# meta-pytorch/torchx

Measured on AMD Instinct MI355X. Metric: tokens_per_second, higher is better.
Workload: dtype bf16; 1 GPU; model=llama3_8b, global_batch=4, seq_len=4096, parallelism=dp1

## Files before the change

torchx_amd/ops/__init__.py:

```python

from __future__ import annotations

import importlib.util
import math
from pathlib import Path
from typing import Optional, Tuple

import torch

from . import reference

_SO = Path(__file__).resolve().parent / "_hip_ops.so"
_hip = None
_load_err: Optional[str] = None


def _load():
    global _hip, _load_err
    if _hip is not None:
        return _hip
    if not _SO.exists():
        _load_err = f"{_SO} not built (run torchx_amd/ops/build.py)"
        return None
    try:
# ... 152 lines not shown
        wt = (hip.transpose_bf16(w)
              if w.shape[0] % 64 == 0 and w.shape[1] % 64 == 0 else None)
        for s in range(0, T, chunk):
            e = min(T, s + chunk)
            x_c = x2[s:e]
            t_c = targets[s:e].contiguous()
            logits_c = x_c @ w.t()
            loss_c, lse_c = hip.ce_fwd(logits_c, t_c)
            loss_sum += loss_c.sum()
            dlog_c = hip.ce_bwd(logits_c, t_c, lse_c, gscale[:e - s])
            if wt is not None:
                torch.matmul(dlog_c, wt.t(), out=dx[s:e])
            else:
                torch.matmul(dlog_c, w, out=dx[s:e])
            if single:
                dw_acc = dlog_c.t() @ x_c
            else:
                dw_acc += dlog_c.t() @ x_c
        ctx.save_for_backward(dx, dw_acc)
        return loss_sum * inv_t

    @staticmethod
    def backward(ctx, gout: torch.Tensor):
        dx, dw_acc = ctx.saved_tensors
        if dw_acc.dtype == dx.dtype:
            dw = dw_acc * gout.to(dx.dtype)
        else:
            dw = (dw_acc * gout.to(torch.float32)).to(dx.dtype)
        dx = dx * gout.to(dx.dtype)
        return dx, dw, None, None


def fused_linear_cross_entropy(
    x: torch.Tensor, w: torch.Tensor, targets: torch.Tensor,
    chunk: int = 16384,
) -> torch.Tensor:
    H = x.shape[-1]
    x2 = x.reshape(-1, H)
    t = targets.reshape(-1)
    if _on_gpu(x):
        if torch.is_grad_enabled() and (x.requires_grad or w.requires_grad):
            return _FusedLinearCE.apply(x2.contiguous(), w, t, chunk)
        hip = hip_ops()
        x2 = x2.contiguous()
        T = x2.shape[0]
        loss_sum = torch.zeros((), device=x.device, dtype=torch.float32)
        for s in range(0, T, chunk):
            e = min(T, s + chunk)
            loss_c, _ = hip.ce_fwd(x2[s:e] @ w.t(), t[s:e].contiguous())
            loss_sum += loss_c.sum()
        return loss_sum / T
    return reference.cross_entropy(x2 @ w.t(), t)




class _FlashAttention(torch.autograd.Function):
    @staticmethod
    def forward(ctx, q: torch.Tensor, k: torch.Tensor, v: torch.Tensor,
                causal: bool, scale: float):
        o, lse = hip_ops().attn_fwd(
            q.contiguous(), k.contiguous(), v.contiguous(), scale, causal
        )
        ctx.save_for_backward(q, k, v, o, lse)
        ctx.causal = causal
        ctx.scale = scale
        return o

    @staticmethod
    def backward(ctx, dout: torch.Tensor):
        q, k, v, o, lse = ctx.saved_tensors
        dq, dk, dv = hip_ops().attn_bwd(
            q, k, v, o, dout.contiguous(), lse, ctx.scale, ctx.causal
        )
        return dq, dk, dv, None, None


def set_attn_bwd_dq_mode(mode: str) -> None:
    hip_ops().set_attn_bwd_dq_mode(mode)


def get_attn_bwd_dq_mode() -> str:
    return hip_ops().get_attn_bwd_dq_mode()


def flash_attention(
    q: torch.Tensor, k: torch.Tensor, v: torch.Tensor,
    causal: bool = True, scale: Optional[float] = None,
) -> torch.Tensor:
    if scale is None:
        scale = 1.0 / math.sqrt(q.shape[-1])
    if _on_gpu(q):
        return _FlashAttention.apply(q, k, v, causal, scale)
    return reference.attention(q, k, v, causal=causal, scale=scale)




def adamw_step(
    p32: torch.Tensor, p16: torch.Tensor, grad: torch.Tensor,
    m: torch.Tensor, v: torch.Tensor, *, lr: float, beta1: float = 0.9,
    beta2: float = 0.95, eps: float = 1e-8, weight_decay: float = 0.1,
    step: int = 1,
) -> None:
    if p32.is_cuda:
        hip_ops().adamw_step(p32, p16, grad, m, v, lr, beta1, beta2, eps,
                             weight_decay, step)
    else:
        reference.adamw_step(p32, p16, grad, m, v, lr=lr, beta1=beta1,
                             beta2=beta2, eps=eps, weight_decay=weight_decay,
                             step=step)


def mfma_probe(a: torch.Tensor, b: torch.Tensor) -> torch.Tensor:
    return hip_ops().mfma_probe(a, b)




class _FastLinear(torch.autograd.Function):
    @staticmethod
    def forward(ctx, x: torch.Tensor, w: torch.Tensor):
        ctx.save_for_backward(x, w)
        return x @ w.t()

    @staticmethod
    def backward(ctx, dy: torch.Tensor):
        x, w = ctx.saved_tensors
        hip = hip_ops()
        wt = hip.transpose_bf16(w)
        dy2 = dy.reshape(-1, dy.shape[-1]).contiguous()
        x2 = x.reshape(-1, x.shape[-1])
        dx = (dy2 @ wt.t()).view_as(x)
        M, N = dy2.shape
        via_t = N <= 8192 and M % 64 == 0 and N % 64 == 0
        wg = w.grad if w.is_leaf else None
        if wg is not None and wg.is_contiguous():
            a = hip.transpose_bf16(dy2) if via_t else dy2.t()
            if getattr(w, "_wgrad_fresh", False):
                torch.matmul(a, x2, out=wg)
                w._wgrad_fresh = False
            else:
                wg.addmm_(a, x2)
            from torchx_amd.parallel.ddp import grad_ready

            grad_ready(w)
            return dx, None
        dw = (hip.transpose_bf16(dy2) @ x2) if via_t else (dy2.t() @ x2)
        return dx, dw


def fast_linear(x: torch.Tensor, w: torch.Tensor) -> torch.Tensor:
    if (x.is_cuda and w.dtype == torch.bfloat16
            and w.shape[0] % 64 == 0 and w.shape[1] % 64 == 0):
        return _FastLinear.apply(x, w)
    return torch.nn.functional.linear(x, w)




class _FusedAttentionQKV(torch.autograd.Function):
    @staticmethod
    def forward(ctx, qkv: torch.Tensor, cos: torch.Tensor, sin: torch.Tensor,
                Hq: int, Hkv: int, causal: bool, scale: float):
        hip = hip_ops()
        roped = hip.rope_qkv(qkv.contiguous(), cos, sin, Hq, Hkv, 1.0, False)
# ... 200 lines not shown
```

torchx_amd/ops/csrc/attention.hip:

```cpp
#include "common.h"

typedef __bf16 mbf16x8 __attribute__((ext_vector_type(8)));

#define HD 128
#define QBLK 32
#define KBLK 32
#define NWAVES 4
#define BLOCK_Q (QBLK * NWAVES)
#define BLOCK_K (KBLK * NWAVES)

__device__ __forceinline__ f32x16 mfma32(mbf16x8 a, mbf16x8 b, f32x16 c) {
  return __builtin_amdgcn_mfma_f32_32x32x16_bf16(a, b, c, 0, 0, 0);
}

__device__ __forceinline__ unsigned int pack_bf16x2(float a, float b) {
  unsigned int r;
  asm("v_cvt_pk_bf16_f32 %0, %1, %2" : "=v"(r) : "v"(a), "v"(b));
  return r;
}

__device__ __forceinline__ int c_row(int r, int half) {
  return (r & 3) + 8 * (r >> 2) + 4 * half;
}

__device__ __forceinline__ void cvals_to_frags(const float* p, bool hi,
                                               mbf16x8* f0, mbf16x8* f1) {
  unsigned int w[2][4];
  #pragma unroll
  for (int s = 0; s < 2; ++s) {
    unsigned int a01 = pack_bf16x2(p[8 * s + 0], p[8 * s + 1]);
    unsigned int a23 = pack_bf16x2(p[8 * s + 2], p[8 * s + 3]);
    unsigned int a45 = pack_bf16x2(p[8 * s + 4], p[8 * s + 5]);
    unsigned int a67 = pack_bf16x2(p[8 * s + 6], p[8 * s + 7]);
    unsigned int x01 = __shfl_xor((int)a01, 32, 64);
    unsigned int x23 = __shfl_xor((int)a23, 32, 64);
    unsigned int x45 = __shfl_xor((int)a45, 32, 64);
    unsigned int x67 = __shfl_xor((int)a67, 32, 64);
    w[s][0] = hi ? x45 : a01;
    w[s][1] = hi ? x67 : a23;
    w[s][2] = hi ? a45 : x01;
    w[s][3] = hi ? a67 : x23;
  }
  uint4_v u0 = {w[0][0], w[0][1], w[0][2], w[0][3]};
  uint4_v u1 = {w[1][0], w[1][1], w[1][2], w[1][3]};
  *f0 = __builtin_bit_cast(mbf16x8, u0);
  *f1 = __builtin_bit_cast(mbf16x8, u1);
}


#define FKV 64
#define KIMG_BYTES (FKV * 256)
#define VIMG_BYTES (HD * FKV * 2)
#define LOG2E 1.44269504088896340736f
#define LN2 0.69314718055994530942f

__device__ __forceinline__ mbf16x8 kimg_frag(const char* kimg, int sub, int c) {
  const int lane = threadIdx.x & 63;
  const int row = sub * 32 + (lane & 31);
  const int byte = (c * 32 + ((lane >> 5) * 16)) ^ ((row & 15) << 4);
  return *(const mbf16x8*)(kimg + row * 256 + byte);
}

__device__ __forceinline__ int vrot(int d) {
  return ((d >> 1) ^ (d >> 4)) & 7;
}

__device__ __forceinline__ mbf16x8 vimg_frag(const char* vimg, int dt, int ks) {
  const int lane = threadIdx.x & 63;
  const int d = dt * 32 + (lane & 31);
  const int g = (ks * 2 + (lane >> 5) + vrot(d)) & 7;
  return *(const mbf16x8*)(vimg + d * 128 + g * 16);
}

typedef short short4_v __attribute__((ext_vector_type(4)));
typedef __attribute__((address_space(3))) short4_v* lds_s4p;

__device__ __forceinline__ mbf16x8 nat_tr_frag(const char* nat, int ks,
                                               int dt) {
  const int lane = threadIdx.x & 63;
  const int j = lane & 15;
  const int r_lo = ks * 16 + ((lane >> 5) * 8) + (j >> 2);
  const int r_hi = r_lo + 4;
  const int d0 = dt * 32 + ((lane >> 4) & 1) * 16 + 4 * (j & 3);
// ... 811 lines not shown
              s2 = -3.0e38f;
            }
          }
          const float pr =
              __builtin_amdgcn_exp2f(s2 - lse_cur[ql]);
          cv[r] = is_dk ? scale * pr * (acc_dp[r] - del_cur[ql]) : pr;
        }

        mbf16x8 f0, f1;
        cvals_to_frags(cv, hi, &f0, &f1);

        const char* acc_img = is_dk ? qn_c : don_c;
        #pragma unroll
        for (int dt = 0; dt < 4; ++dt) {
          acc[dt] =
              mfma32(f0, nat_tr_frag(acc_img, 2 * sb, dt), acc[dt]);
          acc[dt] =
              mfma32(f1, nat_tr_frag(acc_img, 2 * sb + 1, dt), acc[dt]);
          if (dt == 0) {
            __builtin_amdgcn_sched_barrier(0);
            if (ds_on && qs0 < S) {
              char* p = ds_head +
                        (ds_qt_base(qs0 / BLOCK_Q, ds_nqt, causal) * 4 +
                         ((qs0 / QBLK) & 3)) * DS_IMG_BYTES;
              *(uint4_v*)p = __builtin_bit_cast(uint4_v, f0);
              *(uint4_v*)(p + 32) = __builtin_bit_cast(uint4_v, f1);
              n_ds = 2;
            }
          }
        }
      }
    }

    if (has_next) {
      if (n_ds) {
        asm volatile("s_waitcnt vmcnt(2)" ::: "memory");
      } else {
        asm volatile("s_waitcnt vmcnt(0)" ::: "memory");
      }
      stage_lse(ngh, t0 + (idx + 1) % nt_eff, lse_nxt);
      __syncthreads();
      lse_cur = lse_buf[lse_nxt];
      del_cur = del_buf[lse_nxt];
      lse_nxt ^= 1;
      char* tp;
      tp = qn_c; qn_c = qn_n; qn_n = tp;
      tp = don_c; don_c = don_n; don_n = tp;
    }
  }

  unsigned short* out = is_dk ? dk : dv;
  __syncthreads();
  float* tr = (float*)smem + wave * (32 * 36);
  if (wave_active) {
    #pragma unroll
    for (int dt = 0; dt < 4; ++dt) {
      __syncthreads();
      #pragma unroll
      for (int r = 0; r < 16; ++r) {
        tr[c_row(r, hi) * 36 + kr] = acc[dt][r];
      }
      __syncthreads();
      #pragma unroll
      for (int rep = 0; rep < 4; ++rep) {
        const int kk = kr;
        const int d0 = (hi ? 16 : 0) + rep * 4;
        if (kw0 + kk < S) {
          bf16x4_raw w;
          #pragma unroll
          for (int j = 0; j < 4; ++j) {
            w[j] = (short)f32_to_bf16(tr[kk * 36 + d0 + j]);
          }
          *(bf16x4_raw*)(out + ((long)b * S + kw0 + kk) * out_rs +
                         (long)hkv * HD + dt * 32 + d0) = w;
        }
      }
    }
  } else {
    #pragma unroll
    for (int i = 0; i < 8; ++i) __syncthreads();
  }
}

extern "C" void attn_fwd_launch(const void* q, const void* k, const void* v,
                                void* o, void* lse, int B, int S, int Hq,
                                int Hkv, float scale, int causal,
                                long q_rs, long kv_rs, hipStream_t stream) {
  static int fwd8 = -1;
  if (fwd8 < 0) {
    const char* e = getenv("TORCHX_AMD_FWD_8WAVE");
    fwd8 = (e && atoi(e)) ? 1 : 0;
  }
  if (fwd8 == 1) {
    const int nqt = (S + 8 * QBLK - 1) / (8 * QBLK);
    hipLaunchKernelGGL((attn_fwd_kernel<8>), dim3(B * Hq * nqt), dim3(512),
                       0, stream, (const unsigned short*)q,
                       (const unsigned short*)k, (const unsigned short*)v,
                       (unsigned short*)o, (float*)lse, B, S, Hq, Hkv,
                       scale, causal, q_rs, kv_rs);
  } else {
    const int nqt = (S + 4 * QBLK - 1) / (4 * QBLK);
    hipLaunchKernelGGL((attn_fwd_kernel<4>), dim3(B * Hq * nqt), dim3(256),
                       0, stream, (const unsigned short*)q,
                       (const unsigned short*)k, (const unsigned short*)v,
                       (unsigned short*)o, (float*)lse, B, S, Hq, Hkv,
                       scale, causal, q_rs, kv_rs);
  }
}

extern "C" void attn_bwd_launch(const void* q, const void* k, const void* v,
                                const void* o, const void* dout,
                                const void* lse, void* delta, void* dq,
                                void* dk, void* dv, void* ds, int B, int S,
                                int Hq, int Hkv, float scale, int causal,
                                long q_rs, long kv_rs, long dqkv_q_rs,
                                long dqkv_kv_rs, hipStream_t stream) {
  const long rows = (long)B * S * Hq;
  hipLaunchKernelGGL(attn_bwd_pre_kernel, dim3((int)((rows + 15) / 16)),
                     dim3(256), 0, stream, (const unsigned short*)dout,
                     (const unsigned short*)o, (float*)delta, rows, S, Hq);
  const int nkt = (S + BLOCK_K - 1) / BLOCK_K;
  const long dout_rs = (long)Hq * HD;
  static int dkv_fkv = -1;
  if (dkv_fkv < 0) {
    const char* e = getenv("TORCHX_AMD_DKV_FKV");
    dkv_fkv = (e && atoi(e) == 64) ? 64 : 128;
  }
  if (dkv_fkv == 128 && S % 128 == 0) {
    hipLaunchKernelGGL((attn_bwd_dkv_kernel<128>), dim3(B * Hkv * nkt),
                       dim3(512), 0, stream, (const unsigned short*)q,
                       (const unsigned short*)k, (const unsigned short*)v,
                       (const unsigned short*)dout, (const float*)lse,
                       (const float*)delta, (unsigned short*)dk,
                       (unsigned short*)dv, (char*)ds, B, S, Hq, Hkv,
                       scale, causal, q_rs, kv_rs, dout_rs, dqkv_kv_rs);
  } else {
    hipLaunchKernelGGL((attn_bwd_dkv_kernel<64>), dim3(B * Hkv * nkt),
                       dim3(512), 0, stream, (const unsigned short*)q,
                       (const unsigned short*)k, (const unsigned short*)v,
                       (const unsigned short*)dout, (const float*)lse,
                       (const float*)delta, (unsigned short*)dk,
                       (unsigned short*)dv, (char*)ds, B, S, Hq, Hkv,
                       scale, causal, q_rs, kv_rs, dout_rs, dqkv_kv_rs);
  }
  const int nqt = (S + BLOCK_Q - 1) / BLOCK_Q;
  if (ds != nullptr) {
    static int heavy_first = -1;
    if (heavy_first < 0) {
      const char* e = getenv("TORCHX_AMD_DQ_HEAVY_FIRST");
      heavy_first = (e && atoi(e) == 0) ? 0 : 1;
    }
    hipLaunchKernelGGL(attn_bwd_dq_stream_kernel, dim3(B * Hq * nqt),
                       dim3(256), 0, stream, (const unsigned short*)k,
                       (const char*)ds, (unsigned short*)dq, B, S, Hq, Hkv,
                       causal, kv_rs, dqkv_q_rs, heavy_first);
    return;
  }
  static int dq_fkv = -1;
  if (dq_fkv < 0) {
    const char* e = getenv("TORCHX_AMD_DQ_FKV");
    dq_fkv = (e && atoi(e) == 128) ? 128 : 64;
  }
  if (dq_fkv == 128 && S % 128 == 0) {
    hipLaunchKernelGGL((attn_bwd_dq_kernel<128>), dim3(B * Hq * nqt),
                       dim3(256), 0, stream, (const unsigned short*)q,
                       (const unsigned short*)k, (const unsigned short*)v,
                       (const unsigned short*)dout, (const float*)lse,
                       (const float*)delta, (unsigned short*)dq, B, S, Hq,
                       Hkv, scale, causal, q_rs, kv_rs, dqkv_q_rs);
  } else {
    hipLaunchKernelGGL((attn_bwd_dq_kernel<64>), dim3(B * Hq * nqt),
                       dim3(256), 0, stream, (const unsigned short*)q,
                       (const unsigned short*)k, (const unsigned short*)v,
                       (const unsigned short*)dout, (const float*)lse,
                       (const float*)delta, (unsigned short*)dq, B, S, Hq,
                       Hkv, scale, causal, q_rs, kv_rs, dqkv_q_rs);
  }
}
```

torchx_amd/ops/csrc/bindings.cpp:

```cpp
#include <torch/extension.h>
#include <c10/hip/HIPStream.h>

#include <hip/hip_runtime.h>

extern "C" {
void rope_launch(const void*, void*, const void*, const void*, long, int, int,
                 int, float, hipStream_t);
void swiglu_fwd_launch(const void*, const void*, void*, long, hipStream_t);
void swiglu_bwd_launch(const void*, const void*, const void*, void*, void*,
                       long, hipStream_t);
void rmsnorm_fwd_launch(const void*, const void*, void*, void*, long, int,
                        float, hipStream_t);
void rmsnorm_bwd_launch(const void*, const void*, const void*, const void*,
                        void*, void*, void*, long, int, hipStream_t);
long rmsnorm_bwd_dw_chunks(long);
void adamw_launch(void*, void*, const void*, void*, void*, long, float, float,
                  float, float, float, float, float, hipStream_t);
void ce_fwd_launch(const void*, const void*, void*, void*, long, int,
                   hipStream_t);
void ce_bwd_launch(const void*, const void*, const void*, const void*, void*,
                   long, int, hipStream_t);
void attn_fwd_launch(const void*, const void*, const void*, void*, void*, int,
                     int, int, int, float, int, long, long, hipStream_t);
void attn_bwd_launch(const void*, const void*, const void*, const void*,
                     const void*, const void*, void*, void*, void*, void*,
                     void*, int, int, int, int, float, int, long, long, long,
                     long, hipStream_t);
long attn_bwd_ds_bytes(int, int, int, int);
void rope_qkv_launch(const void*, void*, const void*, const void*, long, int,
                     long, int, float, hipStream_t);
void swiglu_gu_fwd_launch(const void*, void*, long, long, hipStream_t);
void swiglu_gu_bwd_launch(const void*, const void*, void*, long, long,
                          hipStream_t);
void mfma_probe_launch(const void*, const void*, void*, hipStream_t);
void mfma_probe_tr_launch(const void*, const void*, void*, void*,
                          hipStream_t);
void fp8_cast_transpose_launch(const void*, void*, void*, void*,
                               const void*, long, long, int, hipStream_t);
void transpose_bf16_launch(const void*, void*, long, long, hipStream_t);
void decode_attn_launch(const void*, const void*, const void*, void*,
                        const void*, int, int, int, int, int, int, float,
                        hipStream_t);
void gemv_bf16_launch(const void*, const void*, void*, int, int, int,
                      hipStream_t);
void decode_attn_split_launch(const void*, const void*, const void*, void*,
                              void*, void*, const void*, int, int, int, int,
                              int, int, int, float, hipStream_t);
void decode_rope_cache_launch(const void*, void*, void*, void*, const void*,
                              const void*, const void*, int, int, int, int,
                              int, int, hipStream_t);
void rmsnorm_res_launch(const void*, const void*, const void*, void*, void*,
                        long, int, float, hipStream_t);
void gemv_swiglu_launch(const void*, const void*, void*, int, int, int,
                        hipStream_t);
void paged_decode_attn_launch(const void*, const void*, const void*, void*,
                              void*, void*, const void*, const void*, int,
                              int, int, int, int, int, int, float,
                              hipStream_t);
void paged_decode_rope_cache_launch(const void*, void*, void*, void*,
                                    const void*, const void*, const void*,
                                    const void*, int, int, int, int, int,
                                    int, int, hipStream_t);
}

namespace {

hipStream_t cur_stream() {
  return c10::hip::getCurrentHIPStream().stream();
}

void check_bf16(const at::Tensor& t, const char* name) {
  TORCH_CHECK(t.is_cuda(), name, " must be on GPU");
  TORCH_CHECK(t.scalar_type() == at::kBFloat16, name, " must be bf16");
  TORCH_CHECK(t.is_contiguous(), name, " must be contiguous");
}

void check_f32(const at::Tensor& t, const char* name) {
  TORCH_CHECK(t.is_cuda(), name, " must be on GPU");
  TORCH_CHECK(t.scalar_type() == at::kFloat, name, " must be f32");
  TORCH_CHECK(t.is_contiguous(), name, " must be contiguous");
}

}

std::vector<at::Tensor> rmsnorm_fwd(at::Tensor x, at::Tensor w, double eps) {
  check_bf16(x, "x");
  check_bf16(w, "w");
  const long H = x.size(-1);
  TORCH_CHECK(H % 2048 == 0 && H <= 8192, "rmsnorm: H must be k*2048, <=8192");
  const long rows = x.numel() / H;
  auto y = at::empty_like(x);
  auto invrms = at::empty({rows}, x.options().dtype(at::kFloat));
  rmsnorm_fwd_launch(x.data_ptr(), w.data_ptr(), y.data_ptr(),
                     invrms.data_ptr(), rows, (int)H, (float)eps,
                     cur_stream());
  return {y, invrms};
}

std::vector<at::Tensor> rmsnorm_bwd(at::Tensor dy, at::Tensor x, at::Tensor w,
                                    at::Tensor invrms) {
  check_bf16(dy, "dy");
  check_bf16(x, "x");
  const long H = x.size(-1);
  TORCH_CHECK(H % 2048 == 0 && H <= 8192, "rmsnorm: H must be k*2048, <=8192");
  const long rows = x.numel() / H;
  auto dx = at::empty_like(x);
  auto dw = at::empty({H}, x.options().dtype(at::kFloat));
  auto dw_part = at::empty({rmsnorm_bwd_dw_chunks(rows), H}, dw.options());
  rmsnorm_bwd_launch(dy.data_ptr(), x.data_ptr(), w.data_ptr(),
                     invrms.data_ptr(), dx.data_ptr(), dw.data_ptr(),
                     dw_part.data_ptr(), rows, (int)H, cur_stream());
// ... 33 lines not shown
                    du.data_ptr(), g.numel(), cur_stream());
  return {dg, du};
}

void adamw_step(at::Tensor p32, at::Tensor p16, at::Tensor g, at::Tensor m,
                at::Tensor v, double lr, double beta1, double beta2,
                double eps, double wd, long step) {
  check_f32(p32, "p32");
  check_bf16(p16, "p16");
  check_bf16(g, "g");
  const long n = p32.numel();
  TORCH_CHECK(n % 4 == 0, "adamw: n must be a multiple of 4");
  const float bc1 = 1.0f - powf((float)beta1, (float)step);
  const float bc2 = 1.0f - powf((float)beta2, (float)step);
  adamw_launch(p32.data_ptr(), p16.data_ptr(), g.data_ptr(), m.data_ptr(),
               v.data_ptr(), n, (float)lr, (float)beta1, (float)beta2,
               (float)eps, (float)wd, bc1, bc2, cur_stream());
}

std::vector<at::Tensor> ce_fwd(at::Tensor logits, at::Tensor targets) {
  check_bf16(logits, "logits");
  TORCH_CHECK(targets.scalar_type() == at::kLong, "targets must be int64");
  const long V = logits.size(-1);
  const long T = logits.numel() / V;
  auto loss = at::empty({T}, logits.options().dtype(at::kFloat));
  auto lse = at::empty({T}, logits.options().dtype(at::kFloat));
  ce_fwd_launch(logits.data_ptr(), targets.data_ptr(), loss.data_ptr(),
                lse.data_ptr(), T, (int)V, cur_stream());
  return {loss, lse};
}

at::Tensor ce_bwd(at::Tensor logits, at::Tensor targets, at::Tensor lse,
                  at::Tensor gscale) {
  check_bf16(logits, "logits");
  check_f32(lse, "lse");
  check_f32(gscale, "gscale");
  const long V = logits.size(-1);
  const long T = logits.numel() / V;
  auto dlogits = at::empty_like(logits);
  ce_bwd_launch(logits.data_ptr(), targets.data_ptr(), lse.data_ptr(),
                gscale.data_ptr(), dlogits.data_ptr(), T, (int)V,
                cur_stream());
  return dlogits;
}

std::vector<at::Tensor> attn_fwd(at::Tensor q, at::Tensor k, at::Tensor v,
                                 double scale, bool causal) {
  check_bf16(q, "q");
  check_bf16(k, "k");
  check_bf16(v, "v");
  const int B = q.size(0), S = q.size(1), Hq = q.size(2), D = q.size(3);
  const int Hkv = k.size(2);
  TORCH_CHECK(D == 128, "attention: head_dim must be 128");
  TORCH_CHECK(Hq % Hkv == 0, "attention: Hq must be a multiple of Hkv");
  auto o = at::empty_like(q);
  auto lse = at::empty({B, Hq, S}, q.options().dtype(at::kFloat));
  attn_fwd_launch(q.data_ptr(), k.data_ptr(), v.data_ptr(), o.data_ptr(),
                  lse.data_ptr(), B, S, Hq, Hkv, (float)scale, causal ? 1 : 0,
                  (long)Hq * 128, (long)Hkv * 128, cur_stream());
  return {o, lse};
}

int g_dq_stream = -1;

bool dq_stream_mode() {
  if (g_dq_stream < 0) {
    const char* e = getenv("TORCHX_AMD_DQ_MODE");
    g_dq_stream = (e && std::string(e) == "recompute") ? 0 : 1;
  }
  return g_dq_stream == 1;
}

void set_attn_bwd_dq_mode(const std::string& mode) {
  TORCH_CHECK(mode == "stream" || mode == "recompute",
              "attn bwd dq mode must be 'stream' or 'recompute', got '",
              mode, "'");
  g_dq_stream = (mode == "stream") ? 1 : 0;
}

std::string get_attn_bwd_dq_mode() {
  return dq_stream_mode() ? "stream" : "recompute";
}

constexpr long kDsScratchCapBytes = 8L << 30;

at::Tensor alloc_ds_scratch(const at::Tensor& like, int B, int S, int Hq,
                            bool causal) {
  if (!dq_stream_mode()) return at::Tensor();
  const long bytes = attn_bwd_ds_bytes(B, S, Hq, causal ? 1 : 0);
  if (bytes > kDsScratchCapBytes) return at::Tensor();
  return at::empty({bytes}, like.options().dtype(at::kByte));
}

std::vector<at::Tensor> attn_bwd(at::Tensor q, at::Tensor k, at::Tensor v,
                                 at::Tensor o, at::Tensor dout, at::Tensor lse,
                                 double scale, bool causal) {
  check_bf16(dout, "dout");
  const int B = q.size(0), S = q.size(1), Hq = q.size(2);
  const int Hkv = k.size(2);
  auto dq = at::empty_like(q);
  auto dk = at::empty_like(k);
  auto dv = at::empty_like(v);
  auto delta = at::empty({B, Hq, S}, q.options().dtype(at::kFloat));
  auto ds = alloc_ds_scratch(q, B, S, Hq, causal);
  attn_bwd_launch(q.data_ptr(), k.data_ptr(), v.data_ptr(), o.data_ptr(),
                  dout.data_ptr(), lse.data_ptr(), delta.data_ptr(),
                  dq.data_ptr(), dk.data_ptr(), dv.data_ptr(),
                  ds.defined() ? ds.data_ptr() : nullptr, B, S, Hq, Hkv,
                  (float)scale, causal ? 1 : 0, (long)Hq * 128,
                  (long)Hkv * 128, (long)Hq * 128, (long)Hkv * 128,
                  cur_stream());
  return {dq, dk, dv};
}

std::vector<at::Tensor> attn_fwd_qkv(at::Tensor qkv, long Hq, long Hkv,
                                     double scale, bool causal) {
  check_bf16(qkv, "qkv");
  const int B = qkv.size(0), S = qkv.size(1);
  const long rs = (Hq + 2 * Hkv) * 128;
  TORCH_CHECK(qkv.size(2) == rs, "qkv last dim mismatch");
  auto o = at::empty({B, S, Hq, 128}, qkv.options());
  auto lse = at::empty({B, Hq, S}, qkv.options().dtype(at::kFloat));
  const unsigned short* base = (const unsigned short*)qkv.data_ptr();
  attn_fwd_launch(base, base + Hq * 128, base + (Hq + Hkv) * 128,
                  o.data_ptr(), lse.data_ptr(), B, S, (int)Hq, (int)Hkv,
                  (float)scale, causal ? 1 : 0, rs, rs, cur_stream());
  return {o, lse};
}

at::Tensor attn_bwd_qkv(at::Tensor qkv, at::Tensor o, at::Tensor dout,
                        at::Tensor lse, long Hq, long Hkv, double scale,
                        bool causal) {
  check_bf16(dout, "dout");
  const int B = qkv.size(0), S = qkv.size(1);
  const long rs = (Hq + 2 * Hkv) * 128;
  auto dqkv = at::empty_like(qkv);
  auto delta = at::empty({B, Hq, S}, qkv.options().dtype(at::kFloat));
  auto ds = alloc_ds_scratch(qkv, B, S, (int)Hq, causal);
  const unsigned short* base = (const unsigned short*)qkv.data_ptr();
  unsigned short* dbase = (unsigned short*)dqkv.data_ptr();
  attn_bwd_launch(base, base + Hq * 128, base + (Hq + Hkv) * 128,
                  o.data_ptr(), dout.data_ptr(), lse.data_ptr(),
                  delta.data_ptr(), dbase, dbase + Hq * 128,
                  dbase + (Hq + Hkv) * 128,
                  ds.defined() ? ds.data_ptr() : nullptr, B, S, (int)Hq,
                  (int)Hkv, (float)scale, causal ? 1 : 0, rs, rs, rs, rs,
                  cur_stream());
  return dqkv;
}

at::Tensor rope_qkv(at::Tensor x, at::Tensor cos_t, at::Tensor sin_t,
                    long Hq, long Hkv, double sign, bool inplace) {
  check_bf16(x, "x");
  check_f32(cos_t, "cos");
  check_f32(sin_t, "sin");
  const int B = x.size(0), S = x.size(1);
  const long rs = (Hq + 2 * Hkv) * 128;
  TORCH_CHECK(x.size(2) == rs, "qkv last dim mismatch");
  at::Tensor y = inplace ? x : at::empty_like(x);
  rope_qkv_launch(x.data_ptr(), y.data_ptr(), cos_t.data_ptr(),
                  sin_t.data_ptr(), (long)B * S, (int)(Hq + Hkv), rs, S,
                  (float)sign, cur_stream());
  if (!inplace) {
    const long v0 = (Hq + Hkv) * 128;
    y.narrow(2, v0, Hkv * 128).copy_(x.narrow(2, v0, Hkv * 128));
  }
// ... 239 lines not shown
  check_f32(sin_t, "sin");
  TORCH_CHECK(qkv.dim() == 2, "qkv must be [B, (Hq+2*Hkv)*128]");
  const int B = qkv.size(0);
  const int logP = check_paged(kpool, vpool, bt, pos, B);
  const int num_pages = kpool.size(0), Hkv = kpool.size(2);
  const int M = bt.size(1);
  TORCH_CHECK(cos_t.dim() == 2 && cos_t.size(1) == 64 &&
                  cos_t.size(0) >= 1 && sin_t.sizes() == cos_t.sizes(),
              "cos/sin must be [S, 64] (head_dim 128)");
  const long nh = qkv.size(1) / 128;
  const int Hq = (int)nh - 2 * Hkv;
  TORCH_CHECK(Hq >= 1 && qkv.size(1) == nh * 128, "qkv width mismatch");
  TORCH_CHECK(Hq % Hkv == 0, "GQA group mismatch");
  const int rope_rows = (int)std::min<long>(cos_t.size(0), 1L << 30);
  auto q = at::empty({B, (long)Hq, 128}, qkv.options());
  paged_decode_rope_cache_launch(qkv.data_ptr(), q.data_ptr(),
                                 kpool.data_ptr(), vpool.data_ptr(),
                                 bt.data_ptr(), cos_t.data_ptr(),
                                 sin_t.data_ptr(), pos.data_ptr(), B, Hq,
                                 Hkv, num_pages, logP, M, rope_rows,
                                 cur_stream());
  return q;
}

std::vector<at::Tensor> rmsnorm_res(at::Tensor x,
                                    c10::optional<at::Tensor> res,
                                    at::Tensor w, double eps) {
  check_bf16(x, "x");
  check_bf16(w, "w");
  const long H = x.size(-1);
  TORCH_CHECK(H % 2048 == 0 && H <= 8192, "rmsnorm: H must be k*2048, <=8192");
  const long R = x.numel() / H;
  auto y = at::empty_like(x);
  at::Tensor s = x;
  const void* rp = nullptr;
  void* sp = nullptr;
  if (res.has_value()) {
    check_bf16(*res, "res");
    TORCH_CHECK(res->sizes() == x.sizes(), "res shape mismatch");
    s = at::empty_like(x);
    rp = res->data_ptr();
    sp = s.data_ptr();
  }
  rmsnorm_res_launch(x.data_ptr(), rp, w.data_ptr(), sp, y.data_ptr(), R,
                     (int)H, (float)eps, cur_stream());
  return {s, y};
}

std::vector<at::Tensor> mfma_probe_tr(at::Tensor a, at::Tensor b) {
  check_bf16(a, "a");
  check_bf16(b, "b");
  TORCH_CHECK(a.size(0) == 32 && a.size(1) == 16, "a must be [32,16]");
  TORCH_CHECK(b.size(0) == 16 && b.size(1) == 32, "b must be [16,32]");
  auto c = at::empty({32, 32}, a.options().dtype(at::kFloat));
  auto raw = at::empty({64, 8}, a.options());
  mfma_probe_tr_launch(a.data_ptr(), b.data_ptr(), c.data_ptr(),
                       raw.data_ptr(), cur_stream());
  return {c, raw};
}

at::Tensor mfma_probe(at::Tensor a, at::Tensor b) {
  check_bf16(a, "a");
  check_bf16(b, "b");
  TORCH_CHECK(a.size(0) == 32 && a.size(1) == 16, "a must be [32,16]");
  TORCH_CHECK(b.size(0) == 16 && b.size(1) == 32, "b must be [16,32]");
  auto c = at::empty({32, 32}, a.options().dtype(at::kFloat));
  mfma_probe_launch(a.data_ptr(), b.data_ptr(), c.data_ptr(), cur_stream());
  return c;
}

PYBIND11_MODULE(TORCH_EXTENSION_NAME, m) {
  m.def("rmsnorm_fwd", &rmsnorm_fwd);
  m.def("rmsnorm_bwd", &rmsnorm_bwd);
  m.def("rope", &rope);
  m.def("swiglu_fwd", &swiglu_fwd);
  m.def("swiglu_bwd", &swiglu_bwd);
  m.def("adamw_step", &adamw_step);
  m.def("ce_fwd", &ce_fwd);
  m.def("ce_bwd", &ce_bwd);
  m.def("attn_fwd", &attn_fwd);
  m.def("attn_bwd", &attn_bwd);
  m.def("set_attn_bwd_dq_mode", &set_attn_bwd_dq_mode);
  m.def("get_attn_bwd_dq_mode", &get_attn_bwd_dq_mode);
  m.def("attn_fwd_qkv", &attn_fwd_qkv);
  m.def("attn_bwd_qkv", &attn_bwd_qkv);
  m.def("rope_qkv", &rope_qkv);
  m.def("swiglu_gu_fwd", &swiglu_gu_fwd);
  m.def("swiglu_gu_bwd", &swiglu_gu_bwd);
  m.def("fp8_cast_transpose", &fp8_cast_transpose);
  m.def("mfma_probe", &mfma_probe);
  m.def("mfma_probe_tr", &mfma_probe_tr);
  m.def("transpose_bf16", &transpose_bf16);
  m.def("decode_attn", &decode_attn);
  m.def("decode_attn_dev", &decode_attn_dev);
  m.def("gemv_bf16", &gemv_bf16);
  m.def("gemv_swiglu_bf16", &gemv_swiglu_bf16);
  m.def("decode_rope_cache", &decode_rope_cache,
        py::arg("qkv"), py::arg("kc"), py::arg("vc"), py::arg("cos"),
        py::arg("sin"), py::arg("pos") = 0,
        py::arg("pos_dev") = c10::nullopt);
  m.def("paged_decode_attn", &paged_decode_attn);
  m.def("paged_decode_rope_cache", &paged_decode_rope_cache);
  m.def("rmsnorm_res", &rmsnorm_res,
        py::arg("x"), py::arg("res"), py::arg("w"), py::arg("eps"));
}
```

Before: 19730 tokens/s.

## Add merged 4-wave dK/dV backward kernel with software-pipelined S/dP chains

Adds a new attention backward dK/dV kernel that uses 256 threads (4 waves) instead of 512, with each wave computing both dV and dK. The next Q sub-block's S and dP MFMA chains are interleaved with the current block's exp/pack stage and transposed-fragment loads, and fragments are repacked with permlane32 swaps. Q/dO tiles, LSE and delta are double-buffered in shared memory. The aim is to raise MFMA utilisation and hide LDS and global latency. It becomes the default, with an env var and setter to fall back to the split kernel. The price is higher register pressure at one block per CU.

After: 21380 tokens/s (median of 6 runs). +8.4%, better.

```diff
diff --git a/torchx_amd/ops/__init__.py b/torchx_amd/ops/__init__.py
--- a/torchx_amd/ops/__init__.py
+++ b/torchx_amd/ops/__init__.py
@@ -258,6 +258,14 @@
 
 def get_attn_bwd_dq_mode() -> str:
     return hip_ops().get_attn_bwd_dq_mode()
+
+
+def set_attn_bwd_dkv_impl(impl: str) -> None:
+    hip_ops().set_attn_bwd_dkv_impl(impl)
+
+
+def get_attn_bwd_dkv_impl() -> str:
+    return hip_ops().get_attn_bwd_dkv_impl()
 
 
 def flash_attention(
diff --git a/torchx_amd/ops/csrc/attention.hip b/torchx_amd/ops/csrc/attention.hip
--- a/torchx_amd/ops/csrc/attention.hip
+++ b/torchx_amd/ops/csrc/attention.hip
@@ -1,4 +1,8 @@
 #include "common.h"
+
+#include <cstdlib>
+#include <cstring>
+#include <type_traits>
 
 typedef __bf16 mbf16x8 __attribute__((ext_vector_type(8)));
 
@@ -976,6 +980,379 @@
   }
 }
 
+__device__ __forceinline__ void packed_to_frags_swap(const unsigned int* a,
+                                                     mbf16x8* f0,
+                                                     mbf16x8* f1) {
+  unsigned int w[2][4];
+  #pragma unroll
+  for (int s = 0; s < 2; ++s) {
+    auto e0 = __builtin_amdgcn_permlane32_swap(a[4 * s + 0], a[4 * s + 2],
+                                               false, false);
+    auto e1 = __builtin_amdgcn_permlane32_swap(a[4 * s + 1], a[4 * s + 3],
+                                               false, false);
+    w[s][0] = e0[0];
+    w[s][1] = e1[0];
+    w[s][2] = e0[1];
+    w[s][3] = e1[1];
+  }
+  uint4_v u0 = {w[0][0], w[0][1], w[0][2], w[0][3]};
+  uint4_v u1 = {w[1][0], w[1][1], w[1][2], w[1][3]};
+  *f0 = __builtin_bit_cast(mbf16x8, u0);
+  *f1 = __builtin_bit_cast(mbf16x8, u1);
+}
+
+template <int TFKV>
+__global__ void __launch_bounds__(256, 1)
+attn_bwd_dkv_merged_kernel(const unsigned short* __restrict__ q,
+                           const unsigned short* __restrict__ k,
+                           const unsigned short* __restrict__ v,
+                           const unsigned short* __restrict__ dout,
+                           const float* __restrict__ lse,
+                           const float* __restrict__ delta,
+                           unsigned short* __restrict__ dk,
+                           unsigned short* __restrict__ dv,
+                           char* __restrict__ ds,
+                           int B, int S, int Hq, int Hkv, float scale,
+                           int causal, long q_rs, long kv_rs, long dout_rs,
+                           long out_rs) {
+  constexpr int NS = TFKV / 32;
+  __shared__ __align__(16) char smem[4 * (TFKV * 256)];
+  __shared__ __align__(16) float lse_buf[2][TFKV], del_buf[2][TFKV];
+  char* qn_c = smem;
+  char* don_c = smem + TFKV * 256;
+  char* qn_n = smem + 2 * (TFKV * 256);
+  char* don_n = smem + 3 * (TFKV * 256);
+
+  const int nkt = (S + BLOCK_K - 1) / BLOCK_K;
+  const int G = Hq / Hkv;
+  int b, hkv, kt;
+  {
+    int bid = blockIdx.x;
+    if (((B * Hkv) & 7) == 0) {
+      const int xcd = bid & 7, slot = bid >> 3;
+      const int g = (slot / nkt) * 8 + xcd;
+      b = g / Hkv;
+      hkv = g % Hkv;
+      kt = slot % nkt;
+    } else {
+      b = bid / (Hkv * nkt);
+      bid -= b * Hkv * nkt;
+      hkv = bid / nkt;
+      kt = bid % nkt;
+    }
+  }
+
+  const int wave = __builtin_amdgcn_readfirstlane(threadIdx.x / 64);
+  const int lane = threadIdx.x & 63;
+  const bool hi = lane >= 32;
+  const int kr = lane & 31;
+
+  const long q_seq_stride = q_rs;
+  const long kv_seq_stride = kv_rs;
+  const unsigned short* kb = k + (long)b * S * kv_seq_stride + (long)hkv * HD;
+  const unsigned short* vb = v + (long)b * S * kv_seq_stride + (long)hkv * HD;
+
+  const int kv0_blk = kt * BLOCK_K;
+  const int kw0 = kv0_blk + wave * KBLK;
+  const long k_row = kw0 + kr;
+  const bool wave_active = kw0 < S;
+  const bool krow_valid = k_row < S;
+
+  mbf16x8 kfrag[8], vfrag[8];
+  {
+    const long row = krow_valid ? k_row : (S - 1);
+    const unsigned short* kp = kb + row * kv_seq_stride + (hi ? 8 : 0);
+    const unsigned short* vp = vb + row * kv_seq_stride + (hi ? 8 : 0);
+    #pragma unroll
+    for (int c = 0; c < 8; ++c) {
+      kfrag[c] = __builtin_bit_cast(mbf16x8, *(const ushort8*)(kp + c * 16));
+      vfrag[c] = __builtin_bit_cast(mbf16x8, *(const ushort8*)(vp + c * 16));
+    }
+  }
+
+  f32x16 accv[4] = {}, acck[4] = {};
+  const float sc2 = scale * LOG2E;
+
+  const int t0 = causal ? (kv0_blk / TFKV) : 0;
+  const int nt = (S + TFKV - 1) / TFKV;
+  const int nt_eff = nt - t0;
+  const int total = G * nt_eff;
+
+  const bool ds_on = ds != nullptr;
+  const int ds_nqt = (S + BLOCK_Q - 1) / BLOCK_Q;
+  const long ds_plane = ds_qt_base(ds_nqt, ds_nqt, causal);
+  const long ds_lane = (long)(kw0 / KBLK) * (4 * DS_IMG_BYTES) + kr * 64 +
+                       (hi ? 16 : 0);
+
+  auto head_q = [&](int gh) {
+    return q + (long)b * S * q_seq_stride + (long)(hkv * G + gh) * HD;
+  };
+  auto head_do = [&](int gh) {
+    return dout + (long)b * S * dout_rs + (long)(hkv * G + gh) * HD;
+  };
+  auto load_lse = [&](int gh, int t) -> float {
+    const int hq_ = hkv * G + gh;
+    const int q0_ = t * TFKV;
+    float x = 0.f;
+    if (threadIdx.x < TFKV) {
+      const float* lse_b = lse + ((long)b * Hq + hq_) * S;
+      const int qg = q0_ + threadIdx.x;
+      x = (qg < S) ? lse_b[qg] : 0.f;
+    } else if (threadIdx.x < 2 * TFKV) {
+      const float* del_b = delta + ((long)b * Hq + hq_) * S;
+      const int qg = q0_ + (threadIdx.x - TFKV);
+      x = (qg < S) ? del_b[qg] : 0.f;
+    }
+    return x;
+  };
+  auto store_lse = [&](int buf, float x) {
+    if (threadIdx.x < TFKV) {
+      lse_buf[buf][threadIdx.x] = x * LOG2E;
+    } else if (threadIdx.x < 2 * TFKV) {
+      del_buf[buf][threadIdx.x - TFKV] = x;
+    }
+  };
+
+  stage_k_glds<4, TFKV>(head_q(0), (long)t0 * TFKV, q_seq_stride, S, qn_c);
+  stage_k_glds<4, TFKV>(head_do(0), (long)t0 * TFKV, dout_rs, S, don_c);
+  asm volatile("s_waitcnt vmcnt(0)");
+  store_lse(0, load_lse(0, t0));
+  __syncthreads();
+
+  const float* lse_cur = lse_buf[0];
+  const float* del_cur = del_buf[0];
+  int lse_nxt = 1;
+  for (int idx = 0; idx < total; ++idx) {
+    const int gh = idx / nt_eff;
+    const int t = t0 + idx % nt_eff;
+    const int q0 = t * TFKV;
+    const int hq = hkv * G + gh;
+    const bool has_next = (idx + 1) < total;
+    const int ngh = (idx + 1) / nt_eff;
+    const int ntile = t0 + (idx + 1) % nt_eff;
+    float lse_reg = 0.f;
+    if (has_next) {
+      stage_k_glds<4, TFKV>(head_q(ngh), (long)ntile * TFKV, q_seq_stride, S,
+                            qn_n);
+      stage_k_glds<4, TFKV>(head_do(ngh), (long)ntile * TFKV, dout_rs, S,
+                            don_n);
+      lse_reg = load_lse(ngh, ntile);
+    }
+
+    int sb0 = 0;
+    if (causal && kw0 > q0) sb0 = (kw0 - q0) / 32;
+    if (!wave_active || sb0 > NS) sb0 = NS;
+    sb0 = __builtin_amdgcn_readfirstlane(sb0);
+
+    int n_ds = 0;
+    char* ds_head = ds + ((long)b * Hq + hq) * ds_plane * (4 * DS_IMG_BYTES)
+                    + ds_lane;
+
+    auto load_frags = [&](int sb, mbf16x8* qf, mbf16x8* of) {
+      #pragma unroll
+      for (int c = 0; c < 8; ++c) {
+        qf[c] = kimg_frag(qn_c, sb, c);
+        of[c] = kimg_frag(don_c, sb, c);
+      }
+    };
+    auto s_chain = [&](const mbf16x8* qf, const mbf16x8* of, f32x16& s_out,
+                       f32x16& dp_out) {
+      f32x16 s = {}, dp = {};
+      #pragma unroll
+      for (int c = 0; c < 8; ++c) {
+        s = mfma32(qf[c], kfrag[c], s);
+        dp = mfma32(of[c], vfrag[c], dp);
+      }
+      s_out = s;
+      dp_out = dp;
+    };
+
+    if (sb0 < NS) {
+      #pragma clang loop unroll(disable)
+      for (int sbase = 0; sbase < NS; sbase += 2) {
+        f32x16 acc_s[2], acc_dp[2];
+        mbf16x8 qf[8], of[8];
+        load_frags(sbase, qf, of);
+        __builtin_amdgcn_sched_barrier(0);
+        s_chain(qf, of, acc_s[0], acc_dp[0]);
+        #pragma unroll
+        for (int u = 0; u < 2; ++u) {
+          const int sb = sbase + u;
+          const bool nx = u == 0;
+          const f32x16& cs = acc_s[u];
+          const f32x16& cdp = acc_dp[u];
+          if (nx) {
+            #pragma unroll
+            for (int c = 0; c < 4; ++c) {
+              qf[c] = kimg_frag(qn_c, sb + 1, c);
+              of[c] = kimg_frag(don_c, sb + 1, c);
+            }
+          }
+          f32x4 lv[4], dl[4];
+          lv[0] = *(const f32x4*)(lse_cur + 32 * sb + (hi ? 4 : 0));
+          dl[0] = *(const f32x4*)(del_cur + 32 * sb + (hi ? 4 : 0));
+          __builtin_amdgcn_sched_barrier(0);
+
+          const int qs0 = q0 + 32 * sb;
+          const bool mask_tile = (causal && qs0 < kw0 + 32)
+                                 || (qs0 + 32 > S) || !krow_valid;
+          mbf16x8 p0, p1, d0, d1;
+          mbf16x8 tv[8], tk[8];
+          auto stage_b = [&](auto masked) {
+            float cp[16], cd[16];
+            unsigned int pp[8], pd[8];
+            f32x16 ns = {}, ndp = {};
+            #pragma unroll
+            for (int r = 0; r < 16; ++r) {
+              if (nx) {
+                if (r & 1) {
+                  ndp = mfma32(of[r >> 1], vfrag[r >> 1], ndp);
+                } else {
+                  ns = mfma32(qf[r >> 1], kfrag[r >> 1], ns);
+                }
+                if (r < 8 && !(r & 1)) {
+                  qf[4 + (r >> 1)] = kimg_frag(qn_c, sb + 1, 4 + (r >> 1));
+                  of[4 + (r >> 1)] = kimg_frag(don_c, sb + 1, 4 + (r >> 1));
+                }
+              }
+              if (r < 12 && !(r & 3)) {
+                const int j = (r >> 2) + 1;
+                lv[j] = *(const f32x4*)(lse_cur + 32 * sb + 8 * j +
+                                        (hi ? 4 : 0));
+                dl[j] = *(const f32x4*)(del_cur + 32 * sb + 8 * j +
+                                        (hi ? 4 : 0));
+              }
+              if (r >= 8) {
+                const int i = r - 8, dt = i >> 2;
+                if (i & 2) {
+                  tk[2 * dt + (i & 1)] =
+                      nat_tr_frag(qn_c, 2 * sb + (i & 1), dt);
+                } else {
+                  tv[2 * dt + (i & 1)] =
+                      nat_tr_frag(don_c, 2 * sb + (i & 1), dt);
+                }
+              }
+              {
+                #pragma clang fp contract(off)
+                const int ql = 32 * sb + c_row(r, hi);
+                float s2 = cs[r] * sc2;
+                if (decltype(masked)::value) {
+                  const long qg = q0 + ql;
+                  if (qg >= S || !krow_valid || (causal && k_row > qg)) {
+                    s2 = -3.0e38f;
+                  }
+                }
+                const float pr =
+                    __builtin_amdgcn_exp2f(s2 - lv[r >> 2][r & 3]);
+                cp[r] = pr;
+                cd[r] = scale * pr * (cdp[r] - dl[r >> 2][r & 3]);
+              }
+              if (r & 1) {
+                pp[r >> 1] = pack_bf16x2(cp[r - 1], cp[r]);
+                pd[r >> 1] = pack_bf16x2(cd[r - 1], cd[r]);
+              }
+              __builtin_amdgcn_sched_barrier(0);
+            }
+            if (nx) {
+              acc_s[1] = ns;
+              acc_dp[1] = ndp;
+            }
+            packed_to_frags_swap(pp, &p0, &p1);
+            packed_to_frags_swap(pd, &d0, &d1);
+          };
+          if (mask_tile) {
+            stage_b(std::true_type{});
+          } else {
+            stage_b(std::false_type{});
+          }
+          __builtin_amdgcn_sched_barrier(0);
+
+          accv[0] = mfma32(p0, tv[0], accv[0]);
+          accv[0] = mfma32(p1, tv[1], accv[0]);
+          acck[0] = mfma32(d0, tk[0], acck[0]);
+          acck[0] = mfma32(d1, tk[1], acck[0]);
+          __builtin_amdgcn_sched_barrier(0);
+          #pragma unroll
+          for (int dt = 2; dt < 4; ++dt) {
+            tv[2 * dt] = nat_tr_frag(don_c, 2 * sb, dt);
+            tv[2 * dt + 1] = nat_tr_frag(don_c, 2 * sb + 1, dt);
+            tk[2 * dt] = nat_tr_frag(qn_c, 2 * sb, dt);
+            tk[2 * dt + 1] = nat_tr_frag(qn_c, 2 * sb + 1, dt);
+          }
+          __builtin_amdgcn_sched_barrier(0);
+          if (ds_on && sb >= sb0 && qs0 < S) {
+            char* p = ds_head +
+                      (ds_qt_base(qs0 / BLOCK_Q, ds_nqt, causal) * 4 +
+                       ((qs0 / QBLK) & 3)) * DS_IMG_BYTES;
+            *(uint4_v*)p = __builtin_bit_cast(uint4_v, d0);
+            *(uint4_v*)(p + 32) = __builtin_bit_cast(uint4_v, d1);
+            n_ds = 2;
+          }
+          __builtin_amdgcn_sched_barrier(0);
+          #pragma unroll
+          for (int dt = 1; dt < 4; ++dt) {
+            accv[dt] = mfma32(p0, tv[2 * dt], accv[dt]);
+            accv[dt] = mfma32(p1, tv[2 * dt + 1], accv[dt]);
+            acck[dt] = mfma32(d0, tk[2 * dt], acck[dt]);
+            acck[dt] = mfma32(d1, tk[2 * dt + 1], acck[dt]);
+          }
+        }
+      }
+    }
+
+    if (has_next) {
+      if (n_ds) {
+        asm volatile("s_waitcnt vmcnt(2)" ::: "memory");
+      } else {
+        asm volatile("s_waitcnt vmcnt(0)" ::: "memory");
+      }
+      store_lse(lse_nxt, lse_reg);
+      asm volatile("s_waitcnt lgkmcnt(0)\n\ts_barrier" ::: "memory");
+      lse_cur = lse_buf[lse_nxt];
+      del_cur = del_buf[lse_nxt];
+      lse_nxt ^= 1;
+      char* tp;
+      tp = qn_c; qn_c = qn_n; qn_n = tp;
+      tp = don_c; don_c = don_n; don_n = tp;
+    }
+  }
+
+  __syncthreads();
+  float* tr = (float*)smem + wave * (32 * 36);
+  if (wave_active) {
+    #pragma unroll
+    for (int o = 0; o < 2; ++o) {
+      unsigned short* out = o ? dk : dv;
+      #pragma unroll
+      for (int dt = 0; dt < 4; ++dt) {
+        __syncthreads();
+        #pragma unroll
+        for (int r = 0; r < 16; ++r) {
+          tr[c_row(r, hi) * 36 + kr] = o ? acck[dt][r] : accv[dt][r];
+        }
+        __syncthreads();
+        #pragma unroll
+        for (int rep = 0; rep < 4; ++rep) {
+          const int kk = kr;
+          const int d0 = (hi ? 16 : 0) + rep * 4;
+          if (kw0 + kk < S) {
+            bf16x4_raw w;
+            #pragma unroll
+            for (int j = 0; j < 4; ++j) {
+              w[j] = (short)f32_to_bf16(tr[kk * 36 + d0 + j]);
+            }
+            *(bf16x4_raw*)(out + ((long)b * S + kw0 + kk) * out_rs +
+                           (long)hkv * HD + dt * 32 + d0) = w;
+          }
+        }
+      }
+    }
+  } else {
+    #pragma unroll
+    for (int i = 0; i < 16; ++i) __syncthreads();
+  }
+}
+
 extern "C" void attn_fwd_launch(const void* q, const void* k, const void* v,
                                 void* o, void* lse, int B, int S, int Hq,
                                 int Hkv, float scale, int causal,
@@ -1000,6 +1377,20 @@
                        (unsigned short*)o, (float*)lse, B, S, Hq, Hkv,
                        scale, causal, q_rs, kv_rs);
   }
+}
+
+static int g_dkv_merged = -1;
+
+extern "C" int attn_bwd_dkv_impl_get() {
+  if (g_dkv_merged < 0) {
+    const char* e = getenv("TORCHX_AMD_DKV_IMPL");
+    g_dkv_merged = (e && strcmp(e, "split") == 0) ? 0 : 1;
+  }
+  return g_dkv_merged;
+}
+
+extern "C" void attn_bwd_dkv_impl_set(int merged) {
+  g_dkv_merged = merged ? 1 : 0;
 }
 
 extern "C" void attn_bwd_launch(const void* q, const void* k, const void* v,
@@ -1020,7 +1411,27 @@
     const char* e = getenv("TORCHX_AMD_DKV_FKV");
     dkv_fkv = (e && atoi(e) == 64) ? 64 : 128;
   }
-  if (dkv_fkv == 128 && S % 128 == 0) {
+  if (attn_bwd_dkv_impl_get() == 1) {
+    if (dkv_fkv == 128 && S % 128 == 0) {
+      hipLaunchKernelGGL((attn_bwd_dkv_merged_kernel<128>),
+                         dim3(B * Hkv * nkt), dim3(256), 0, stream,
+                         (const unsigned short*)q, (const unsigned short*)k,
+                         (const unsigned short*)v,
+                         (const unsigned short*)dout, (const float*)lse,
+                         (const float*)delta, (unsigned short*)dk,
+                         (unsigned short*)dv, (char*)ds, B, S, Hq, Hkv,
+                         scale, causal, q_rs, kv_rs, dout_rs, dqkv_kv_rs);
+    } else {
+      hipLaunchKernelGGL((attn_bwd_dkv_merged_kernel<64>),
+                         dim3(B * Hkv * nkt), dim3(256), 0, stream,
+                         (const unsigned short*)q, (const unsigned short*)k,
+                         (const unsigned short*)v,
+                         (const unsigned short*)dout, (const float*)lse,
+                         (const float*)delta, (unsigned short*)dk,
+                         (unsigned short*)dv, (char*)ds, B, S, Hq, Hkv,
+                         scale, causal, q_rs, kv_rs, dout_rs, dqkv_kv_rs);
+    }
+  } else if (dkv_fkv == 128 && S % 128 == 0) {
     hipLaunchKernelGGL((attn_bwd_dkv_kernel<128>), dim3(B * Hkv * nkt),
                        dim3(512), 0, stream, (const unsigned short*)q,
                        (const unsigned short*)k, (const unsigned short*)v,
diff --git a/torchx_amd/ops/csrc/bindings.cpp b/torchx_amd/ops/csrc/bindings.cpp
--- a/torchx_amd/ops/csrc/bindings.cpp
+++ b/torchx_amd/ops/csrc/bindings.cpp
@@ -27,6 +27,8 @@
                      void*, int, int, int, int, float, int, long, long, long,
                      long, hipStream_t);
 long attn_bwd_ds_bytes(int, int, int, int);
+int attn_bwd_dkv_impl_get();
+void attn_bwd_dkv_impl_set(int);
 void rope_qkv_launch(const void*, void*, const void*, const void*, long, int,
                      long, int, float, hipStream_t);
 void swiglu_gu_fwd_launch(const void*, void*, long, long, hipStream_t);
@@ -226,6 +228,17 @@
   return dq_stream_mode() ? "stream" : "recompute";
 }
 
+void set_attn_bwd_dkv_impl(const std::string& impl) {
+  TORCH_CHECK(impl == "merged" || impl == "split",
+              "attn bwd dkv impl must be 'merged' or 'split', got '", impl,
+              "'");
+  attn_bwd_dkv_impl_set(impl == "merged" ? 1 : 0);
+}
+
+std::string get_attn_bwd_dkv_impl() {
+  return attn_bwd_dkv_impl_get() == 1 ? "merged" : "split";
+}
+
 constexpr long kDsScratchCapBytes = 8L << 30;
 
 at::Tensor alloc_ds_scratch(const at::Tensor& like, int B, int S, int Hq,
@@ -631,6 +644,8 @@
   m.def("attn_bwd", &attn_bwd);
   m.def("set_attn_bwd_dq_mode", &set_attn_bwd_dq_mode);
   m.def("get_attn_bwd_dq_mode", &get_attn_bwd_dq_mode);
+  m.def("set_attn_bwd_dkv_impl", &set_attn_bwd_dkv_impl);
+  m.def("get_attn_bwd_dkv_impl", &get_attn_bwd_dkv_impl);
   m.def("attn_fwd_qkv", &attn_fwd_qkv);
   m.def("attn_bwd_qkv", &attn_bwd_qkv);
   m.def("rope_qkv", &rope_qkv);
```
